# LuoGroup2023/PanTax

Measured on AMD Instinct MI355X. Metric: PAO wall-time (s) + Mreads/s: packed reads + DB (graphs and their unique-trio index) resident in HBM -> abundance tables; the metric's own GAF -> abundance quantity is value_gaf_to_tables (files -> tables, never `value`), higher is better.
Workload: dtype int64+f64

## Files before the change

include/pantax_hip.h:

```cpp
#ifndef PANTAX_HIP_H
#define PANTAX_HIP_H
#include <stddef.h>
#include <stdint.h>
#ifdef __cplusplus
extern "C" {
#endif

typedef enum {
    PANTAX_HIP_OK = 0,
    PANTAX_HIP_E_INVALID = -1,
    PANTAX_HIP_E_HIP = -2,
    PANTAX_HIP_E_NO_DEVICE = -3,
    PANTAX_HIP_E_LIMIT = -4,
    PANTAX_HIP_E_SOLVER = -5,
    PANTAX_HIP_E_IO = -6,
    PANTAX_HIP_E_STATE = -7
} pantax_hip_status;

typedef struct pantax_hip_ctx pantax_hip_ctx;
typedef struct pantax_hip_db pantax_hip_db;
typedef struct pantax_hip_reads pantax_hip_reads;

int pantax_hip_init(pantax_hip_ctx **out, const int *device_ids, int n_devices);
void pantax_hip_destroy(pantax_hip_ctx *ctx);
int pantax_hip_set_option(pantax_hip_ctx *ctx, const char *name, const char *value);
const char *pantax_hip_last_error(const pantax_hip_ctx *ctx);
const char *pantax_hip_version(void);

typedef struct {
    uint32_t n_species;
    const int64_t *range_start;
    const int64_t *range_end;
    const uint64_t *node_off;
    const int64_t *node_len;
    const uint64_t *hap_off;
    const uint64_t *path_off;
    const uint32_t *path_nodes;
} pantax_hip_graphs;

int pantax_hip_db_upload(pantax_hip_ctx *ctx, const pantax_hip_graphs *g, pantax_hip_db **out);
// ... 229 lines not shown
```

pantax_amd/_ffi.py:

```python
import ctypes as C
import os

import numpy as np

_HERE = os.path.dirname(os.path.abspath(__file__))
LIB_PATH = os.path.join(_HERE, "lib", "libpantax_hip.so")
_lib = None

SYMBOLS = [
    "pantax_hip_init", "pantax_hip_destroy", "pantax_hip_last_error", "pantax_hip_version", "pantax_hip_set_option",
    "pantax_hip_db_upload", "pantax_hip_db_upload_parts", "pantax_hip_db_free", "pantax_hip_reads_upload", "pantax_hip_reads_free",
    "pantax_hip_bin_reads", "pantax_hip_species_profile", "pantax_hip_db_reset", "pantax_hip_abundance_filter",
    "pantax_hip_trio_index", "pantax_hip_trio_get", "pantax_hip_node_coverage",
    "pantax_hip_strain_profile", "pantax_hip_strain_node_stats", "pantax_hip_strain_hap_stats", "pantax_hip_pao_solve", "pantax_hip_pao_solve_batch", "pantax_hip_profile", "pantax_hip_profile_step", "pantax_hip_profile_step_enqueue", "pantax_hip_profile_step_collect", "pantax_hip_trio_index_prefetch", "pantax_hip_sort_rows",
    "pantax_hip_sample_ranks", "pantax_hip_chacha_block", "pantax_hip_gaf_filter", "pantax_hip_db_save_images", "pantax_hip_db_load_images",
    "pantax_hip_gaf_load", "pantax_hip_gaf_load_device", "pantax_hip_reads_load_gaf", "pantax_hip_reads_set_flags", "pantax_hip_gaf_view", "pantax_hip_gaf_free",
    "pantax_hip_graph_load", "pantax_hip_graph_view", "pantax_hip_graph_free", "pantax_hip_format_f64",
    "pantax_hip_read_strains", "pantax_hip_reads_route_pack", "pantax_hip_route_buffer", "pantax_hip_route_free", "pantax_hip_reads_from_routed",
    "pantax_hip_timing_enable", "pantax_hip_timing_filter", "pantax_hip_timing_reset", "pantax_hip_timing_get", "pantax_hip_sync",
]


class PantaxHipError(RuntimeError):
    def __init__(self, code, msg):
        super().__init__("pantax_hip error %d: %s" % (code, msg))
# ... 73 lines not shown
ALLREDUCE_FN = C.CFUNCTYPE(C.c_int, C.c_void_p, C.POINTER(C.c_double), C.c_uint64)
ALLTOALLV_FN = C.CFUNCTYPE(C.c_int, C.c_void_p, C.c_void_p, C.POINTER(C.c_uint64), C.c_void_p, C.POINTER(C.c_uint64))


def load():
    global _lib
    if _lib is None:
        path = os.environ.get("PANTAX_HIP_LIB") or LIB_PATH
        if not os.path.exists(path):
            raise ImportError("%s is not built (run `python -c 'import __graft_entry__ as g; g.build()'`); "
                              "pantax_amd has no CPU fallback" % path)
        _lib = C.CDLL(path)
        _lib.pantax_hip_last_error.restype = C.c_char_p
        _lib.pantax_hip_last_error.argtypes = [C.c_void_p]
        _lib.pantax_hip_version.restype = C.c_char_p
        _lib.pantax_hip_destroy.restype = None
        _lib.pantax_hip_db_free.restype = None
        _lib.pantax_hip_reads_free.restype = None
        _lib.pantax_hip_gaf_free.restype = None
        _lib.pantax_hip_graph_free.restype = None
        _lib.pantax_hip_route_free.restype = None
        _lib.pantax_hip_read_strains.restype = C.c_int
        _lib.pantax_hip_read_strains.argtypes = [C.c_void_p, C.c_void_p, C.c_void_p, C.POINTER(ReadStrainSet), C.c_void_p, C.c_void_p, C.c_void_p]
    return _lib


def p(a):
    return None if a is None else a.ctypes.data_as(C.c_void_p)


# ... 3 lines not shown
```

pantax_amd/csrc/common.hpp:

```cpp
#pragma once
#include <hip/hip_runtime.h>
#include <cstdint>
#include <cstdio>
#include <map>
#include <functional>
#include <mutex>
#include <cstring>
#include <atomic>
#include <string>
#include <vector>
#include "../../include/pantax_hip.h"

#ifndef TRIO_LH_PACK
#define TRIO_LH_PACK 0
#endif
namespace ptx {

struct Ctx;
#if TRIO_LH_PACK
using trio_len_t = uint2;
#else
using trio_len_t = uint32_t;
#endif

// ... 101 lines not shown
    std::string cov_long;
    int covl_shape = -1;
    bool cov_count = false;
    int cov_clean_async = -1;
    bool cov_self_clean = false;
    bool walk_sum_in_bin = false;
    int ncs_prefix_min = 48;
    bool ncs_no_prefix = false;
    bool cov_arena_verify = false;
    int cov_item_groups = 0;
    int tv_u = 4, tv_rounds = 4, tf_u = 8, tf_rounds = 1, rows_u = 1, tb_slots = 256, trio_xcd = 3, cov_shape = -1, covf_shape = -1, cov_xcd = 0, group_bucket_bits = 0;
    uint32_t tv_ablate = 0, cov_ablate = 0, ssn_ablate = 0;
    bool trio_two_pass = false;
    std::string bin_route;
    std::string node_pass;
    bool no_absent_skip = false;
    bool ssn_debug = false, scan_no_huge = false, flag_rank_chained = false, ratio_kernel = false, mask_pass = false, trio_free_at_filter = false,
         trio_after_step = false;
};
int ctx_set_option(CtxConfig &cfg, const char *name, const char *value);

struct NumaInfo {
    int node = -1;
    std::vector<int> cpus;
};

struct Ctx {
    std::recursive_mutex mu;
    CtxConfig cfg;
    NumaInfo numa;
// ... 422 lines not shown
```

pantax_amd/csrc/ctx.cpp:

```cpp
#include <exception>
#include <cstdarg>
#include <algorithm>
#include <atomic>
#include <cstring>
#include <functional>
#include <chrono>
#include <condition_variable>
#include <cstdio>
#include <mutex>
#include <thread>
#include <unistd.h>
#include <fcntl.h>
#include <sched.h>
#include <pthread.h>
#include <sys/syscall.h>
#include <fstream>
#include <cctype>
#include <cstddef>
#include <cstdlib>
#include "common.hpp"

namespace ptx {

static thread_local std::string g_init_err;
static thread_local std::string g_thread_err;
static thread_local const Ctx *g_thread_err_ctx = nullptr;

int fail(Ctx *ctx, int code, const char *fmt, ...) {
    char buf[1024];
    va_list ap;
    va_start(ap, fmt);
    vsnprintf(buf, sizeof(buf), fmt, ap);
    va_end(ap);
    if (ctx) {
        { std::lock_guard<std::mutex> g(ctx->err_mu); ctx->err = buf; }
// ... 45 lines not shown
    ctx->pending.clear();
    return 0;
}

namespace {
enum OptKind { O_BOOL, O_INT, O_U32, O_U64, O_STR };
struct OptDesc { const char *name; OptKind kind; size_t off; };
#define OPT(nm, kind, field) {nm, kind, offsetof(CtxConfig, field)}
const OptDesc OPTIONS[] = {
    OPT("hip_trace", O_BOOL, trace), OPT("stage_threads", O_INT, stage_threads), OPT("stage_ch_mb", O_INT, stage_ch_mb), OPT("stream_prio", O_BOOL, stream_prio), OPT("numa_bind", O_BOOL, numa_bind), OPT("dev_cache_gb", O_INT, dev_cache_gb),
    OPT("gaf_piece_bytes", O_U64, gaf_piece_bytes), OPT("db_path_steps_max", O_U64, db_path_steps_max), OPT("db_groups", O_INT, db_groups), OPT("trio_path", O_STR, trio_path), OPT("trio_rows", O_STR, trio_rows), OPT("trio_two_pass", O_BOOL, trio_two_pass), OPT("uniq_hash", O_INT, uniq_hash),
    OPT("mask", O_STR, mask), OPT("row_sort", O_STR, row_sort), OPT("objective", O_STR, objective), OPT("read_strain_route", O_STR, read_strain_route),
    OPT("cov_general", O_BOOL, cov_general), OPT("cov_long", O_STR, cov_long), OPT("covl_shape", O_INT, covl_shape), OPT("cov_count", O_BOOL, cov_count), OPT("cov_self_clean", O_BOOL, cov_self_clean), OPT("cov_clean_async", O_INT, cov_clean_async), OPT("cov_arena_verify", O_BOOL, cov_arena_verify), OPT("ncs_no_prefix", O_BOOL, ncs_no_prefix), OPT("ncs_prefix_min", O_INT, ncs_prefix_min), OPT("walk_sum_in_bin", O_BOOL, walk_sum_in_bin), OPT("cov_item_groups", O_INT, cov_item_groups), OPT("tv_u", O_INT, tv_u), OPT("tv_rounds", O_INT, tv_rounds), OPT("tf_u", O_INT, tf_u), OPT("tf_rounds", O_INT, tf_rounds),
    OPT("rows_u", O_INT, rows_u), OPT("tb_slots", O_INT, tb_slots), OPT("trio_xcd", O_INT, trio_xcd), OPT("cov_shape", O_INT, cov_shape),
    OPT("covf_shape", O_INT, covf_shape), OPT("cov_xcd", O_INT, cov_xcd), OPT("group_bucket_bits", O_INT, group_bucket_bits), OPT("tv_ablate", O_U32, tv_ablate),
    OPT("cov_ablate", O_U32, cov_ablate), OPT("ssn_ablate", O_U32, ssn_ablate), OPT("no_absent_skip", O_BOOL, no_absent_skip), OPT("node_pass", O_STR, node_pass), OPT("bin_route", O_STR, bin_route), OPT("ssn_debug", O_BOOL, ssn_debug),
    OPT("scan_no_huge", O_BOOL, scan_no_huge), OPT("flag_rank_chained", O_BOOL, flag_rank_chained), OPT("ratio_kernel", O_BOOL, ratio_kernel),
    OPT("mask_pass", O_BOOL, mask_pass), OPT("trio_free_at_filter", O_BOOL, trio_free_at_filter), OPT("trio_after_step", O_BOOL, trio_after_step),
};
#undef OPT
}

int ctx_set_option(CtxConfig &cfg, const char *name, const char *value) {
    if (!name) return PANTAX_HIP_E_INVALID;
    static const CtxConfig defaults;
    for (const OptDesc &o : OPTIONS) {
        if (std::strcmp(o.name, name) != 0) continue;
        char *dst = reinterpret_cast<char *>(&cfg) + o.off;
        const char *def = reinterpret_cast<const char *>(&defaults) + o.off;
        char *end = nullptr;
        switch (o.kind) {
// ... 20 lines not shown

}

using namespace ptx;

extern "C" {

const char *pantax_hip_version(void) { return "pantax-hip 0.1.0 (gfx950)"; }

int pantax_hip_set_option(pantax_hip_ctx *ctx, const char *name, const char *value) {
    if (!ctx || !name) return PANTAX_HIP_E_INVALID;
    std::lock_guard<std::recursive_mutex> ptx_lock__(ctx->mu);
    const int rc = ctx_set_option(ctx->cfg, name, value);
    if (rc == 0 && std::strcmp(name, "dev_cache_gb") == 0) dev_cache_set_max(ctx->cfg.dev_cache_gb < 0 ? -1 : (long long)ctx->cfg.dev_cache_gb << 30);
    return rc == 0 ? 0 : fail(ctx, rc, "set_option: unknown option or unparsable value: %s=%s", name, value ? value : "(default)");
}

const char *pantax_hip_last_error(const pantax_hip_ctx *ctx) {
    if (!ctx) return g_init_err.c_str();
    if (g_thread_err_ctx == ctx) return g_thread_err.c_str();
    std::lock_guard<std::mutex> g(const_cast<pantax_hip_ctx *>(ctx)->err_mu);
    g_thread_err = ctx->err;
    return g_thread_err.c_str();
}

int pantax_hip_init(pantax_hip_ctx **out, const int *device_ids, int n_devices) {
    if (!out) return PANTAX_HIP_E_INVALID;
    *out = nullptr;
    if (n_devices != 1) return fail(nullptr, PANTAX_HIP_E_INVALID, "one ctx drives one GPU (one process per GPU); n_devices=%d", n_devices);
    int count = 0;
// ... 551 lines not shown
```

pantax_amd/csrc/lad.hpp:

```cpp
#pragma once
#include "common.hpp"

namespace ptx {

int hap_trio_stats_launch(Ctx *ctx, Db *db, DevBuf<uint32_t> &d_ntrio_nz , DevBuf<double> &d_mean ,
                          const uint8_t *d_active = nullptr );
int node_stats_launch(Ctx *ctx, Db *db, LadBatch *lb, int64_t min_depth, const uint8_t *d_active = nullptr);
struct RowRoute {
    uint64_t max_vs;
    uint32_t max_haps;
    bool wide;
    bool by_node;
    bool use_nodes;
    bool use_sample;
    bool ratio_by_node;
    bool masks_in_sort;
};
RowRoute row_route(const Ctx *ctx, const Db *db);
int row_pack_shift(const RowRoute &rt, uint32_t S, int pmax_bound);
bool node_pass_fused_eligible(const Ctx *ctx, const Db *db, const pantax_hip_strain_config *cfg);
int row_sample_apply(Ctx *ctx, const Db *db, LadBatch *lb, int64_t sample_nodes);
int lad_prepare(Ctx *ctx, Db *db, LadBatch *lb, bool cand_on_device, int pmax_bound);
int lad_solve_launch(Ctx *ctx, const Db *db, LadBatch *lb, int pmax_bound, const uint8_t *d_need, const uint8_t *d_fixed, double *d_x,
                     double *d_obj, int32_t *d_status, int32_t *d_iters);
struct FilterCfg;
int lad_pair_launch(Ctx *ctx, const Db *db, LadBatch *lb, int pmax_bound, const FilterCfg &fc);
int objective_launch(Ctx *ctx, const Db *db, LadBatch *lb, const uint8_t *d_need2, const double *d_x1, const double *d_x2, double *d_obj1, double *d_obj2);
struct FilterCfg { double fr, fc, sr; int shift; };
int first_filter_launch(Ctx *ctx, const Db *db, LadBatch *lb, const uint8_t *d_active, const FilterCfg &fc);

int strain_prezero(Ctx *ctx, Db *db);
int strain_enqueue(Ctx *ctx, Db *db, const pantax_hip_strain_config *cfg, const uint8_t *d_active, int slot);
int strain_finish(Ctx *ctx, Db *db, const pantax_hip_strain_config *cfg, const uint8_t *species_active, const double *species_coverage,
                  pantax_hip_hap_metrics *met, pantax_hip_solve_info *info_out, void (*after_wait)(void *), void *after_wait_arg, int slot);
int trio_index_build(Ctx *ctx, Db *db, bool with_keys);
// ... 3 lines not shown
```

pantax_amd/csrc/stage_lad.hip:

```cpp
#include <algorithm>
#include <cstdio>
#include <vector>
#include "lad.hpp"
#include "lad_device.hpp"
#include "second_filter.hpp"
#include "primitives.hpp"
#include "wave.hpp"

namespace ptx {

__device__ __forceinline__ uint32_t lower_bound_a(const double *__restrict__ a, uint32_t lo, uint32_t hi, double v) {
    while (lo < hi) { uint32_t m = (lo + hi) >> 1; if (a[m] < v) lo = m + 1; else hi = m; }
    return lo;
}
__device__ __forceinline__ uint32_t upper_bound_a(const double *__restrict__ a, uint32_t lo, uint32_t hi, double v) {
    while (lo < hi) { uint32_t m = (lo + hi) >> 1; if (a[m] <= v) lo = m + 1; else hi = m; }
    return lo;
}
__device__ __forceinline__ uint32_t wave_bound(const double *__restrict__ a, uint32_t lo, uint32_t hi, double v, bool upper) {
    const uint32_t lane = threadIdx.x & 63;
    while (hi - lo > 64) {
        const uint32_t m = hi - lo;
        const uint32_t pj = lo + (uint32_t)(((uint64_t)(lane + 1) * m) / 65);
        const double x = a[pj];
// ... 45 lines not shown
            const uint32_t jj = coop ? wave_bound(r.idx, j0, j1, v, upper)
                                     : (upper ? upper_bound_a(r.idx, j0, j1, v) : lower_bound_a(r.idx, j0, j1, v));
            if (jj > j0) lo = r.row0 + ((jj - 1) << r.shift) + 1;
            if (jj < j1) hi = r.row0 + (jj << r.shift);
        }
    }
    if (coop) return wave_bound(r.a, lo, hi, v, upper);
    return upper ? upper_bound_a(r.a, lo, hi, v) : lower_bound_a(r.a, lo, hi, v);
}
__device__ __forceinline__ uint32_t lb(bool coop, const RowIdx &r, uint32_t lo, uint32_t hi, double v) { return bound_idx(coop, r, lo, hi, v, false); }
__device__ __forceinline__ uint32_t ub_(bool coop, const RowIdx &r, uint32_t lo, uint32_t hi, double v) { return bound_idx(coop, r, lo, hi, v, true); }

constexpr int LAD_BLOCK = 256;
constexpr int LAD_KWIDE = 16;
constexpr int LAD_KLDS = 256;
enum { C_LB = 0, C_UB = 1, C_PAT = 2, C_FIXED = 3 };

#ifdef LAD_PROFILE
#define LAD_TICK(ph) do { if (tid == 0 && A.prof) { const unsigned long long now_ = wall_clock64(); A.prof[(size_t)s * 16 + (ph)] += now_ - t_prev_; \
                                                     A.prof[(size_t)s * 16 + 8 + (ph)] += 1; t_prev_ = now_; } } while (0)
#else
#define LAD_TICK(ph) do { } while (0)
#endif
struct LadArgs {
    unsigned long long *prof;
    const double *row_a;
    const uint64_t *pat_mask;
    const uint32_t *pat_start;
    const uint32_t *sp_pat_off;
    double *pat_eps, *sc_s, *sc_rho;
// ... 57 lines not shown
                off += n;                                                                                                  \
            }                                                                                                              \
            L_coff[k1 - k0] = off;                                                                                         \
        }                                                                                                                  \
        __syncthreads();                                                                                                   \
        const uint32_t total = L_coff[k1 - k0];                                                                            \
        for (uint32_t e = tid; e < total; e += LAD_BLOCK) {                                                                \
            uint32_t kk = 0, kh = k1 - k0;     \
            while (kh - kk > 1) { const uint32_t km_ = (kk + kh) >> 1; if (L_coff[km_] <= e) kk = km_; else kh = km_; }         \
            L_cache[e] = ra.a[L_crow0[kk] + (e - L_coff[kk])];                                                             \
        }                                                                                                                  \
        __syncthreads();                                                                                                   \
        cached = true;                                                                                                     \
    }
#define PAT_LOOP(k) for (uint32_t k = k0 + (COOP ? (uint32_t)(tid >> 6) : (uint32_t)tid); k < k1; k += (COOP ? LAD_BLOCK / 64 : LAD_BLOCK))
template <int PS, int NW>
struct LadLds {
    static constexpr uint32_t IDX_N = PS <= 16 ? 4096 : 2048;
    static constexpr bool CACHE_IN_G = NW == 1 && PS > 16;
    static constexpr uint32_t CACHE_N = PS <= 16 ? 2048 : CACHE_IN_G ? PS * 2 * PS : 512;
    LadShared<PS> sh;
    double W[NW == 1 ? PS * PS : 1];
    double G[NW == 1 ? PS * 2 * PS : 1];
    double L_s[LAD_KLDS], L_rho[LAD_KLDS], L_eps[LAD_KLDS];
    uint64_t L_mask[LAD_KLDS];
    uint32_t L_lo[LAD_KLDS], L_up[LAD_KLDS], L_lslo[LAD_KLDS], L_lshi[LAD_KLDS], L_lsmid[LAD_KLDS], L_start[LAD_KLDS + 1];
    double L_idx[IDX_N];
    double L_cache[CACHE_IN_G ? 1 : CACHE_N];
    uint32_t L_lsmid2[LAD_KLDS], L_coff[LAD_KLDS + 1], L_cn[LAD_KLDS], L_crow0[LAD_KLDS];
    uint32_t W_cmin[LAD_KWIDE][64], W_cmax[LAD_KWIDE][64];
    double W_acc[LAD_BLOCK / 64][2][64];
};

template <int PS, bool USEL, int NW>
__device__ __forceinline__ void lad_solve_body(const LadArgs &A, LadLds<PS, NW> &m, const int s, const int p, const uint32_t k0, const uint32_t k1) {
    static_assert(NW == 1 || !USEL, "wide species keep their pattern state in global scratch");
    constexpr uint32_t IDX_N = LadLds<PS, NW>::IDX_N, CACHE_N = LadLds<PS, NW>::CACHE_N;
    constexpr bool HUGE = NW == 0;
    const int nw = HUGE ? (int)A.wide_nw[s] : NW;
    const int ps = HUGE ? 64 * nw : PS;
    LadShared<PS> &sh = m.sh;
    double *W, *G;
    const uint64_t *patw = nullptr;
    double *q_x, *q_c, *q_d, *q_ub, *q_fac, *q_score, *q_deriv;
    long long *q_g;
    int *q_type, *q_jk, *q_dir;
    uint32_t *q_i0, *q_i1;
    if constexpr (NW == 1) { W = m.W; G = m.G; }
    else {
        const uint64_t wo = A.wide_woff[A.wide_slot[s]];
        W = A.wide_W + wo; G = A.wide_G + 2 * wo;
        patw = A.pat_or + (size_t)A.wide_off[s] * LAD_WIDE_NW;
// ... 3 lines not shown
        int *i32 = A.huge_i32 + (size_t)A.wide_coff[A.wide_slot[s]] * 5;
        q_x = f; q_c = f + ps; q_d = f + 2 * ps; q_ub = f + 3 * ps; q_fac = f + 4 * ps; q_score = f + 5 * ps; q_deriv = f + 6 * ps;
        q_g = reinterpret_cast<long long *>(f + 7 * (size_t)ps);
        q_type = i32; q_jk = i32 + ps; q_dir = i32 + 2 * ps;
        q_i0 = reinterpret_cast<uint32_t *>(i32 + 3 * (size_t)ps); q_i1 = reinterpret_cast<uint32_t *>(i32 + 4 * (size_t)ps);
    } else {
        q_x = sh.x; q_c = sh.c; q_d = sh.d; q_ub = sh.ub; q_fac = sh.fac; q_score = sh.score; q_deriv = sh.deriv; q_g = sh.g;
        q_type = sh.act_type; q_jk = sh.act_jk; q_dir = sh.dir; q_i0 = sh.act_i0; q_i1 = sh.act_i1;
    }
    auto slot_of_pattern = [&](uint32_t k) -> int {
        if constexpr (HUGE) return A.pat_act[k];
        else { int ai = -1; for (int i = 0; i < p; ++i) if (q_type[i] == C_PAT && (uint32_t)q_jk[i] == k) ai = i; return ai; }
    };
    const uint64_t c0 = A.col_off[s];
    double *L_s = m.L_s, *L_rho = m.L_rho, *L_eps = m.L_eps, *L_idx = m.L_idx, *L_cache;
    if constexpr (LadLds<PS, NW>::CACHE_IN_G) L_cache = m.G; else L_cache = m.L_cache;
    uint64_t *L_mask = m.L_mask;
    uint32_t *L_lo = m.L_lo, *L_up = m.L_up, *L_lslo = m.L_lslo, *L_lshi = m.L_lshi, *L_lsmid = m.L_lsmid, *L_start = m.L_start,
             *L_lsmid2 = m.L_lsmid2, *L_coff = m.L_coff, *L_cn = m.L_cn, *L_crow0 = m.L_crow0;
    uint32_t (*W_cmin)[64] = m.W_cmin, (*W_cmax)[64] = m.W_cmax;
    double (*W_acc)[2][64] = m.W_acc;
    const int tid = threadIdx.x;
    const bool COOP = (k1 - k0) <= (uint32_t)LAD_KWIDE;
    const bool leader = COOP ? ((tid & 63) == 0) : true;
    constexpr bool useL = USEL;
    const uint32_t kofs = useL ? k0 : 0u;
    double *P_sc_s = useL ? L_s : A.sc_s, *P_sc_rho = useL ? L_rho : A.sc_rho, *P_pat_eps = useL ? L_eps : A.pat_eps;
    uint32_t *P_sc_lo = useL ? L_lo : A.sc_lo, *P_sc_up = useL ? L_up : A.sc_up, *P_ls_lo = useL ? L_lslo : A.ls_lo,
             *P_ls_hi = useL ? L_lshi : A.ls_hi, *P_ls_mid = useL ? L_lsmid : A.ls_mid;
    const uint64_t *P_pat_mask = useL ? L_mask : A.pat_mask;
    const uint32_t *P_pat_start = useL ? L_start : A.pat_start;
// ... 641 lines not shown
        if (v > q_ub[j]) v = q_ub[j];
        A.x_out[c0 + j] = v;
    }
    if (tid == 0) {
        A.status[s] = (it >= max_it) ? 1 : sh.status;
        A.iters[s] = it;
    }
}

template <int NW>
__device__ __forceinline__ bool lad_instance_takes(const LadArgs &A, int s, int p) {
    if (NW == 1) return p <= LAD_MAXP;
    if (p <= LAD_MAXP) return false;
    return (NW == 0) == (A.wide_nw[s] > (uint32_t)LAD_WIDE_NW);
}
template <int PS, int NW>
__global__ void __launch_bounds__(LAD_BLOCK) lad_solve_kernel(LadArgs A) {
    __shared__ LadLds<PS, NW> m;
    const int s = NW == 1 ? (int)blockIdx.x : (int)A.wide_list[blockIdx.x];
    const int p = A.sp_p[s];
    if (!lad_instance_takes<NW>(A, s, p)) return;
    if (A.need && !A.need[s]) return;
    if (p <= 0) { if (threadIdx.x == 0) { A.status[s] = 0; A.iters[s] = 0; } return; }
    const uint32_t k0 = A.sp_pat_off[s], k1 = A.sp_pat_off[s + 1];
    if constexpr (NW == 1) {
        if (k1 - k0 <= (uint32_t)LAD_KLDS) lad_solve_body<PS, true, 1>(A, m, s, p, k0, k1);
        else lad_solve_body<PS, false, 1>(A, m, s, p, k0, k1);
    } else lad_solve_body<PS, false, NW>(A, m, s, p, k0, k1);
}

template <int PS, int NW>
__global__ void __launch_bounds__(LAD_BLOCK) lad_pair_kernel(LadArgs A1, LadArgs A2, SecondFilterArgs F) {
    __shared__ LadLds<PS, NW> m;
    const int s = NW == 1 ? (int)blockIdx.x : (int)A1.wide_list[blockIdx.x];
    const int p = A1.sp_p[s];
    if (!lad_instance_takes<NW>(A1, s, p)) return;
    const uint32_t k0 = A1.sp_pat_off[s], k1 = A1.sp_pat_off[s + 1];
    const bool lds_state = NW == 1 && k1 - k0 <= (uint32_t)LAD_KLDS;
    if (p > 0) {
        if constexpr (NW == 1) {
            if (lds_state) lad_solve_body<PS, true, 1>(A1, m, s, p, k0, k1);
            else lad_solve_body<PS, false, 1>(A1, m, s, p, k0, k1);
        } else lad_solve_body<PS, false, NW>(A1, m, s, p, k0, k1);
    } else if (threadIdx.x == 0) { A1.status[s] = 0; A1.iters[s] = 0; }
    __syncthreads();
    if (threadIdx.x == 0) second_filter_species(F, (uint32_t)s);
    __syncthreads();
    if (p <= 0 || !F.need2[s]) return;
    if constexpr (NW == 1) {
        if (lds_state) lad_solve_body<PS, true, 1>(A2, m, s, p, k0, k1);
        else lad_solve_body<PS, false, 1>(A2, m, s, p, k0, k1);
    } else lad_solve_body<PS, false, NW>(A2, m, s, p, k0, k1);
}

static SecondFilterArgs second_filter_args(const Db *db, LadBatch *lb, const FilterCfg &fc, const double *d_x1, const int32_t *d_status1,
                                           uint8_t *d_fixed2, uint8_t *d_need2) {
    SecondFilterArgs F;
    F.hap_off = db->d_hap_off.p; F.hap_nt = lb->d_hap_nt.p; F.sp_trio = lb->d_sp_trio.p; F.hap_bit = lb->d_hap_bit.p; F.sp_p = lb->d_p.p; F.nnz = db->d_hap_nnz.p;
    F.meanf = db->d_hap_mean.p; F.ratio = lb->d_ratio.p; F.x1 = d_x1; F.status1 = d_status1; F.fc = fc.fc; F.sr = fc.sr;
    F.fixed2 = d_fixed2; F.need2 = d_need2;
    return F;
}
static LadArgs lad_args(const Db *db, LadBatch *lb, const uint8_t *d_need, const uint8_t *d_fixed, double *d_x, int32_t *d_status, int32_t *d_iters) {
    LadArgs A;
    A.prof = nullptr;
    A.row_a = lb->row_a; A.pat_mask = lb->d_pat_mask.p; A.pat_start = lb->d_pat_start.p; A.sp_pat_off = lb->d_sp_pat_off.p;
    A.pat_eps = lb->d_pat_eps.p; A.sc_s = lb->d_sc_s.p; A.sc_rho = lb->d_sc_rho.p;
// ... 25 lines not shown
    for (uint32_t s = 0; s < S && s < 4; ++s) {
        unsigned long long tot = 0;
        for (int ph = 0; ph < 8; ++ph) tot += h[(size_t)s * 16 + ph];
        if (!tot) continue;
        std::fprintf(stderr, "[lad profile] species %u: %d pivots, %.1f us in the pivot loop (%.1f us per pivot)\n", s, it[s], tot * 0.01, it[s] ? tot * 0.01 / it[s] : 0.0);
        for (int ph = 0; ph < 8; ++ph)
            std::fprintf(stderr, "    %-22s %9.1f us  %5.1f %%  (%llu visits, %.2f us each)\n", LAD_PHASE_NAMES[ph], h[(size_t)s * 16 + ph] * 0.01,
                         100.0 * h[(size_t)s * 16 + ph] / tot, h[(size_t)s * 16 + 8 + ph], h[(size_t)s * 16 + 8 + ph] ? h[(size_t)s * 16 + ph] * 0.01 / h[(size_t)s * 16 + 8 + ph] : 0.0);
    }
    return 0;
}
#endif

int lad_pair_launch(Ctx *ctx, const Db *db, LadBatch *lb, int pmax_bound, const FilterCfg &fc) {
    const uint32_t S = db->S;
    LadArgs A1 = lad_args(db, lb, nullptr, nullptr, lb->d_x.p, lb->d_status.p, lb->d_iters.p);
    LadArgs A2 = lad_args(db, lb, nullptr, lb->d_fixed2.p, lb->d_x2.p, lb->d_status2.p, lb->d_iters2.p);
    SecondFilterArgs F = second_filter_args(db, lb, fc, lb->d_x.p, lb->d_status.p, lb->d_fixed2.p, lb->d_need2.p);
#ifdef LAD_PROFILE
    DevBuf<unsigned long long> prof;
    PTX_TRY(lad_prof_begin(ctx, S, prof, A1));
#endif
    {
        KTimer t(ctx, "lad_pair_kernel");
        if (pmax_bound <= 16) hipLaunchKernelGGL((lad_pair_kernel<16, 1>), dim3(S), dim3(LAD_BLOCK), 0, ctx->stream, A1, A2, F);
        else hipLaunchKernelGGL((lad_pair_kernel<LAD_MAXP, 1>), dim3(S), dim3(LAD_BLOCK), 0, ctx->stream, A1, A2, F);
        if (lb->n_wide > lb->n_huge) hipLaunchKernelGGL((lad_pair_kernel<LAD_WIDEP, LAD_WIDE_NW>), dim3(lb->n_wide), dim3(LAD_BLOCK), 0, ctx->stream, A1, A2, F);
        if (lb->n_huge) hipLaunchKernelGGL((lad_pair_kernel<1, 0>), dim3(lb->n_wide), dim3(LAD_BLOCK), 0, ctx->stream, A1, A2, F);
    }
    PTX_HIP(ctx, hipGetLastError());
#ifdef LAD_PROFILE
    PTX_TRY(lad_prof_end(ctx, S, prof, lb->d_iters.p));
#endif
    return objective_launch(ctx, db, lb, lb->d_need2.p, lb->d_x.p, lb->d_x2.p, lb->d_obj.p, lb->d_obj2.p);
}

int lad_solve_launch(Ctx *ctx, const Db *db, LadBatch *lb, int pmax_bound, const uint8_t *d_need, const uint8_t *d_fixed, double *d_x,
                     double *d_obj, int32_t *d_status, int32_t *d_iters) {
    const uint32_t S = db->S;
    LadArgs A = lad_args(db, lb, d_need, d_fixed, d_x, d_status, d_iters);
#ifdef LAD_PROFILE
    DevBuf<unsigned long long> prof;
    PTX_TRY(lad_prof_begin(ctx, S, prof, A));
#endif
    {
        KTimer t(ctx, "lad_solve_kernel");
        if (pmax_bound <= 16) hipLaunchKernelGGL((lad_solve_kernel<16, 1>), dim3(S), dim3(LAD_BLOCK), 0, ctx->stream, A);
        else hipLaunchKernelGGL((lad_solve_kernel<LAD_MAXP, 1>), dim3(S), dim3(LAD_BLOCK), 0, ctx->stream, A);
        if (lb->n_wide > lb->n_huge) hipLaunchKernelGGL((lad_solve_kernel<LAD_WIDEP, LAD_WIDE_NW>), dim3(lb->n_wide), dim3(LAD_BLOCK), 0, ctx->stream, A);
        if (lb->n_huge) hipLaunchKernelGGL((lad_solve_kernel<1, 0>), dim3(lb->n_wide), dim3(LAD_BLOCK), 0, ctx->stream, A);
    }
    PTX_HIP(ctx, hipGetLastError());
#ifdef LAD_PROFILE
    PTX_TRY(lad_prof_end(ctx, S, prof, d_iters));
#endif
    return objective_launch(ctx, db, lb, nullptr, d_x, nullptr, d_obj, nullptr);
}

}
```

pantax_amd/csrc/stage_lp_rows.hip:

```cpp
#include <algorithm>
#include <cstdio>
#include <vector>
#include "lad.hpp"
#include "lad_device.hpp"
#include "primitives.hpp"
#include "wave.hpp"
#include "scan_chained.hpp"

namespace ptx {

__device__ __forceinline__ uint32_t find_hap_l(const uint64_t *__restrict__ path_off, uint32_t H, uint64_t q) {
    uint32_t lo = 0, hi = H;
    while (lo < hi) { uint32_t mid = (lo + hi) >> 1; if (path_off[mid] <= q) lo = mid + 1; else hi = mid; }
    return lo - 1;
}

__global__ void __launch_bounds__(256) mask_kernel(const uint2 *__restrict__ tiles, const uint64_t *__restrict__ path_off,
                                                   const uint32_t *__restrict__ path_nodes, const uint32_t *__restrict__ hap_species,
                                                   const uint32_t *__restrict__ node_base, const int32_t *__restrict__ hap_bit,
                                                   unsigned long long *__restrict__ mask, const int32_t *__restrict__ sp_p,
                                                   const uint32_t *__restrict__ wide_off ,
                                                   const uint32_t *__restrict__ wide_nw, unsigned long long *__restrict__ maskw,
                                                   const uint64_t *__restrict__ by_node_hap_off ) {
    const uint2 tile = tiles[blockIdx.x];
// ... 440 lines not shown
        if (ev[0] == 'n') r.use_nodes = r.max_vs <= SSN_MAX_SEG && S <= 65535 && V > 0;
    }
    r.use_sample = V <= SS_MAX_N;
    r.by_node = use_node_haps(ctx, db);
    r.ratio_by_node = r.by_node && V && !ctx->cfg.ratio_kernel;
    r.wide = max_hs > (uint64_t)LAD_MAXP;
    const bool mask_pass_env = ctx->cfg.mask_pass || ctx->cfg.objective == "nodes";
    r.masks_in_sort = r.use_nodes && r.ratio_by_node && !db->nh_walk_too && !r.wide && !mask_pass_env;
    return r;
}
int row_pack_shift(const RowRoute &rt, uint32_t S, int pmax_bound) {
    const int sp_bits = S > 1 ? bits_for(S - 1) : 0;
    return (!rt.use_sample && sp_bits + pmax_bound <= 64 && !(rt.use_nodes && pmax_bound >= 64)) ? pmax_bound : -1;
}

bool node_pass_fused_eligible(const Ctx *ctx, const Db *db, const pantax_hip_strain_config *cfg) {
    if (ctx->cfg.node_pass == "split" || !db->cov_count_pending || db->V == 0) return false;
    if (cfg->sample_nodes != 0 || ctx->cfg.cov_self_clean || db->cov_self_clean) return false;
    if (db->L / db->V >= (uint64_t)ctx->cfg.ncs_prefix_min && !ctx->cfg.ncs_no_prefix) return false;
    return row_route(ctx, db).masks_in_sort;
}

static int upload_candidates(Ctx *ctx, const Db *db, LadBatch *lb) {
    const uint32_t S = db->S;
    const uint64_t H = db->H;
    std::vector<int32_t> hap_bit(H ? H : 1, -1);
    for (uint32_t s = 0; s < S; ++s)
        for (int k = 0; k < lb->h_p[s]; ++k) hap_bit[db->h_hap_off[s] + lb->h_cand[db->h_hap_off[s] + k]] = k;
    PTX_TRY(upload(ctx, lb->d_hap_bit, hap_bit.data(), hap_bit.size()));
    PTX_TRY(upload(ctx, lb->d_p, lb->h_p.data(), S));
// ... 195 lines not shown
```

pantax_amd/engine.py:

```python
import ctypes as C

import numpy as np

from . import _ffi
from ._ffi import PantaxHipError, as_c, p


class Engine:
    def __init__(self, device=0):
        self.lib = _ffi.load()
        self.ctx = C.c_void_p()
        dev = (C.c_int * 1)(device)
        rc = self.lib.pantax_hip_init(C.byref(self.ctx), dev, 1)
        if rc != 0:
            raise PantaxHipError(rc, self.lib.pantax_hip_last_error(None).decode())
        self.db = None
        self.reads = None
        self._keep = []
        self._step_buf = None
        self._collect_buf = None
        self._inflight = 0

    def _check(self, rc):
        if rc != 0:
# ... 21 lines not shown
                self.lib.pantax_hip_db_free(self.ctx, self.db)
                self.db = None
            self._inflight = 0

    def __enter__(self):
        return self

    def __exit__(self, *a):
        self.close()

    def sync(self):
        self._check(self.lib.pantax_hip_sync(self.ctx))

    def set_option(self, name, value=None):
        self._check(self.lib.pantax_hip_set_option(self.ctx, name.encode(), None if value is None else str(value).encode()))

    def upload_db(self, species):
        if self.db:
            self.lib.pantax_hip_db_free(self.ctx, self.db)
            self.db = None
            self._inflight = 0
        S = len(species)
        self.S = S
        self.range_start = as_c([g.range_start for g in species], np.int64)
        self.range_end = as_c([g.range_end for g in species], np.int64)
        self.node_off = np.zeros(S + 1, dtype=np.uint64)
        self.node_off[1:] = np.cumsum([len(g.node_len) for g in species])
        self.hap_off = np.zeros(S + 1, dtype=np.uint64)
        self.hap_off[1:] = np.cumsum([len(g.path_off) - 1 for g in species])
        self.V = int(self.node_off[-1])
# ... 476 lines not shown
```

Baseline: 6284.

## Add compact LDS shape for 16-column LAD solver when species exceed CUs

Adds a second shared-memory layout for the 16-column LAD solver kernels with smaller index, cache and per-pattern LDS arrays plus a waves-per-EU hint of 4. By default it is chosen automatically when there are more species workgroups than compute units, so several workgroups can share a CU instead of one large-LDS block each. The trade-off is that species with more than 32 patterns fall back to the global-memory state path, and index and cache capacity shrink, which may cost extra global traffic. An option and a query function expose the choice.

```diff
diff --git a/include/pantax_hip.h b/include/pantax_hip.h
--- a/include/pantax_hip.h
+++ b/include/pantax_hip.h
@@ -24,6 +24,7 @@
 int pantax_hip_init(pantax_hip_ctx **out, const int *device_ids, int n_devices);
 void pantax_hip_destroy(pantax_hip_ctx *ctx);
 int pantax_hip_set_option(pantax_hip_ctx *ctx, const char *name, const char *value);
+const char *pantax_hip_lad_shape_name(const pantax_hip_ctx *ctx, uint32_t n_species, int max_columns);
 const char *pantax_hip_last_error(const pantax_hip_ctx *ctx);
 const char *pantax_hip_version(void);
 
diff --git a/pantax_amd/_ffi.py b/pantax_amd/_ffi.py
--- a/pantax_amd/_ffi.py
+++ b/pantax_amd/_ffi.py
@@ -8,7 +8,7 @@
 _lib = None
 
 SYMBOLS = [
-    "pantax_hip_init", "pantax_hip_destroy", "pantax_hip_last_error", "pantax_hip_version", "pantax_hip_set_option",
+    "pantax_hip_init", "pantax_hip_destroy", "pantax_hip_last_error", "pantax_hip_version", "pantax_hip_set_option", "pantax_hip_lad_shape_name",
     "pantax_hip_db_upload", "pantax_hip_db_upload_parts", "pantax_hip_db_free", "pantax_hip_reads_upload", "pantax_hip_reads_free",
     "pantax_hip_bin_reads", "pantax_hip_species_profile", "pantax_hip_db_reset", "pantax_hip_abundance_filter",
     "pantax_hip_trio_index", "pantax_hip_trio_get", "pantax_hip_node_coverage",
@@ -112,6 +112,8 @@
         _lib.pantax_hip_last_error.restype = C.c_char_p
         _lib.pantax_hip_last_error.argtypes = [C.c_void_p]
         _lib.pantax_hip_version.restype = C.c_char_p
+        _lib.pantax_hip_lad_shape_name.restype = C.c_char_p
+        _lib.pantax_hip_lad_shape_name.argtypes = [C.c_void_p, C.c_uint32, C.c_int]
         _lib.pantax_hip_destroy.restype = None
         _lib.pantax_hip_db_free.restype = None
         _lib.pantax_hip_reads_free.restype = None
diff --git a/pantax_amd/csrc/common.hpp b/pantax_amd/csrc/common.hpp
--- a/pantax_amd/csrc/common.hpp
+++ b/pantax_amd/csrc/common.hpp
@@ -139,6 +139,7 @@
     bool trio_two_pass = false;
     std::string bin_route;
     std::string node_pass;
+    std::string lad_shape;
     bool no_absent_skip = false;
     bool ssn_debug = false, scan_no_huge = false, flag_rank_chained = false, ratio_kernel = false, mask_pass = false, trio_free_at_filter = false,
          trio_after_step = false;
diff --git a/pantax_amd/csrc/ctx.cpp b/pantax_amd/csrc/ctx.cpp
--- a/pantax_amd/csrc/ctx.cpp
+++ b/pantax_amd/csrc/ctx.cpp
@@ -19,6 +19,7 @@
 #include <cstddef>
 #include <cstdlib>
 #include "common.hpp"
+#include "lad.hpp"
 
 namespace ptx {
 
@@ -94,7 +95,7 @@
     OPT("cov_general", O_BOOL, cov_general), OPT("cov_long", O_STR, cov_long), OPT("covl_shape", O_INT, covl_shape), OPT("cov_count", O_BOOL, cov_count), OPT("cov_self_clean", O_BOOL, cov_self_clean), OPT("cov_clean_async", O_INT, cov_clean_async), OPT("cov_arena_verify", O_BOOL, cov_arena_verify), OPT("ncs_no_prefix", O_BOOL, ncs_no_prefix), OPT("ncs_prefix_min", O_INT, ncs_prefix_min), OPT("walk_sum_in_bin", O_BOOL, walk_sum_in_bin), OPT("cov_item_groups", O_INT, cov_item_groups), OPT("tv_u", O_INT, tv_u), OPT("tv_rounds", O_INT, tv_rounds), OPT("tf_u", O_INT, tf_u), OPT("tf_rounds", O_INT, tf_rounds),
     OPT("rows_u", O_INT, rows_u), OPT("tb_slots", O_INT, tb_slots), OPT("trio_xcd", O_INT, trio_xcd), OPT("cov_shape", O_INT, cov_shape),
     OPT("covf_shape", O_INT, covf_shape), OPT("cov_xcd", O_INT, cov_xcd), OPT("group_bucket_bits", O_INT, group_bucket_bits), OPT("tv_ablate", O_U32, tv_ablate),
-    OPT("cov_ablate", O_U32, cov_ablate), OPT("ssn_ablate", O_U32, ssn_ablate), OPT("no_absent_skip", O_BOOL, no_absent_skip), OPT("node_pass", O_STR, node_pass), OPT("bin_route", O_STR, bin_route), OPT("ssn_debug", O_BOOL, ssn_debug),
+    OPT("cov_ablate", O_U32, cov_ablate), OPT("ssn_ablate", O_U32, ssn_ablate), OPT("no_absent_skip", O_BOOL, no_absent_skip), OPT("node_pass", O_STR, node_pass), OPT("bin_route", O_STR, bin_route), OPT("lad_shape", O_STR, lad_shape), OPT("ssn_debug", O_BOOL, ssn_debug),
     OPT("scan_no_huge", O_BOOL, scan_no_huge), OPT("flag_rank_chained", O_BOOL, flag_rank_chained), OPT("ratio_kernel", O_BOOL, ratio_kernel),
     OPT("mask_pass", O_BOOL, mask_pass), OPT("trio_free_at_filter", O_BOOL, trio_free_at_filter), OPT("trio_after_step", O_BOOL, trio_after_step),
 };
@@ -145,6 +146,11 @@
     const int rc = ctx_set_option(ctx->cfg, name, value);
     if (rc == 0 && std::strcmp(name, "dev_cache_gb") == 0) dev_cache_set_max(ctx->cfg.dev_cache_gb < 0 ? -1 : (long long)ctx->cfg.dev_cache_gb << 30);
     return rc == 0 ? 0 : fail(ctx, rc, "set_option: unknown option or unparsable value: %s=%s", name, value ? value : "(default)");
+}
+
+const char *pantax_hip_lad_shape_name(const pantax_hip_ctx *ctx, uint32_t n_species, int max_columns) {
+    if (!ctx) return nullptr;
+    return lad_shape_name(lad_shape(ctx->cfg.lad_shape, n_species, ctx->n_cu, max_columns));
 }
 
 const char *pantax_hip_last_error(const pantax_hip_ctx *ctx) {
diff --git a/pantax_amd/csrc/lad.hpp b/pantax_amd/csrc/lad.hpp
--- a/pantax_amd/csrc/lad.hpp
+++ b/pantax_amd/csrc/lad.hpp
@@ -19,6 +19,9 @@
 RowRoute row_route(const Ctx *ctx, const Db *db);
 int row_pack_shift(const RowRoute &rt, uint32_t S, int pmax_bound);
 bool node_pass_fused_eligible(const Ctx *ctx, const Db *db, const pantax_hip_strain_config *cfg);
+enum class LadShape { roomy, compact };
+LadShape lad_shape(const std::string &option, uint32_t n_workgroups, int n_cu, int pmax_bound);
+const char *lad_shape_name(LadShape s);
 int row_sample_apply(Ctx *ctx, const Db *db, LadBatch *lb, int64_t sample_nodes);
 int lad_prepare(Ctx *ctx, Db *db, LadBatch *lb, bool cand_on_device, int pmax_bound);
 int lad_solve_launch(Ctx *ctx, const Db *db, LadBatch *lb, int pmax_bound, const uint8_t *d_need, const uint8_t *d_fixed, double *d_x,
diff --git a/pantax_amd/csrc/stage_lad.hip b/pantax_amd/csrc/stage_lad.hip
--- a/pantax_amd/csrc/stage_lad.hip
+++ b/pantax_amd/csrc/stage_lad.hip
@@ -83,6 +83,9 @@
 constexpr int LAD_BLOCK = 256;
 constexpr int LAD_KWIDE = 16;
 constexpr int LAD_KLDS = 256;
+
+struct LadRoomy { static constexpr uint32_t IDX_N = 4096, CACHE_N = 2048; static constexpr int KLDS = LAD_KLDS, WAVES = 1; };
+struct LadCompact { static constexpr uint32_t IDX_N = 1024, CACHE_N = 1024; static constexpr int KLDS = 32, WAVES = 4; };
 enum { C_LB = 0, C_UB = 1, C_PAT = 2, C_FIXED = 3 };
 
 #ifdef LAD_PROFILE
@@ -170,28 +173,30 @@
         cached = true;                                                                                                     \
     }
 #define PAT_LOOP(k) for (uint32_t k = k0 + (COOP ? (uint32_t)(tid >> 6) : (uint32_t)tid); k < k1; k += (COOP ? LAD_BLOCK / 64 : LAD_BLOCK))
-template <int PS, int NW>
+template <int PS, int NW, class SH = LadRoomy>
 struct LadLds {
-    static constexpr uint32_t IDX_N = PS <= 16 ? 4096 : 2048;
+    static_assert(PS <= 16 || SH::KLDS == LAD_KLDS, "only the 16-column instance has more than one shape");
+    static constexpr int KLDS = SH::KLDS;
+    static constexpr uint32_t IDX_N = PS <= 16 ? SH::IDX_N : 2048;
     static constexpr bool CACHE_IN_G = NW == 1 && PS > 16;
-    static constexpr uint32_t CACHE_N = PS <= 16 ? 2048 : CACHE_IN_G ? PS * 2 * PS : 512;
+    static constexpr uint32_t CACHE_N = PS <= 16 ? SH::CACHE_N : CACHE_IN_G ? PS * 2 * PS : 512;
     LadShared<PS> sh;
     double W[NW == 1 ? PS * PS : 1];
     double G[NW == 1 ? PS * 2 * PS : 1];
-    double L_s[LAD_KLDS], L_rho[LAD_KLDS], L_eps[LAD_KLDS];
-    uint64_t L_mask[LAD_KLDS];
-    uint32_t L_lo[LAD_KLDS], L_up[LAD_KLDS], L_lslo[LAD_KLDS], L_lshi[LAD_KLDS], L_lsmid[LAD_KLDS], L_start[LAD_KLDS + 1];
+    double L_s[KLDS], L_rho[KLDS], L_eps[KLDS];
+    uint64_t L_mask[KLDS];
+    uint32_t L_lo[KLDS], L_up[KLDS], L_lslo[KLDS], L_lshi[KLDS], L_lsmid[KLDS], L_start[KLDS + 1];
     double L_idx[IDX_N];
     double L_cache[CACHE_IN_G ? 1 : CACHE_N];
-    uint32_t L_lsmid2[LAD_KLDS], L_coff[LAD_KLDS + 1], L_cn[LAD_KLDS], L_crow0[LAD_KLDS];
+    uint32_t L_lsmid2[KLDS], L_coff[KLDS + 1], L_cn[KLDS], L_crow0[KLDS];
     uint32_t W_cmin[LAD_KWIDE][64], W_cmax[LAD_KWIDE][64];
     double W_acc[LAD_BLOCK / 64][2][64];
 };
 
-template <int PS, bool USEL, int NW>
-__device__ __forceinline__ void lad_solve_body(const LadArgs &A, LadLds<PS, NW> &m, const int s, const int p, const uint32_t k0, const uint32_t k1) {
+template <int PS, bool USEL, int NW, class SH>
+__device__ __forceinline__ void lad_solve_body(const LadArgs &A, LadLds<PS, NW, SH> &m, const int s, const int p, const uint32_t k0, const uint32_t k1) {
     static_assert(NW == 1 || !USEL, "wide species keep their pattern state in global scratch");
-    constexpr uint32_t IDX_N = LadLds<PS, NW>::IDX_N, CACHE_N = LadLds<PS, NW>::CACHE_N;
+    constexpr uint32_t IDX_N = LadLds<PS, NW, SH>::IDX_N, CACHE_N = LadLds<PS, NW, SH>::CACHE_N;
     constexpr bool HUGE = NW == 0;
     const int nw = HUGE ? (int)A.wide_nw[s] : NW;
     const int ps = HUGE ? 64 * nw : PS;
@@ -225,7 +230,7 @@
     };
     const uint64_t c0 = A.col_off[s];
     double *L_s = m.L_s, *L_rho = m.L_rho, *L_eps = m.L_eps, *L_idx = m.L_idx, *L_cache;
-    if constexpr (LadLds<PS, NW>::CACHE_IN_G) L_cache = m.G; else L_cache = m.L_cache;
+    if constexpr (LadLds<PS, NW, SH>::CACHE_IN_G) L_cache = m.G; else L_cache = m.L_cache;
     uint64_t *L_mask = m.L_mask;
     uint32_t *L_lo = m.L_lo, *L_up = m.L_up, *L_lslo = m.L_lslo, *L_lshi = m.L_lshi, *L_lsmid = m.L_lsmid, *L_start = m.L_start,
              *L_lsmid2 = m.L_lsmid2, *L_coff = m.L_coff, *L_cn = m.L_cn, *L_crow0 = m.L_crow0;
@@ -897,9 +902,9 @@
     if (p <= LAD_MAXP) return false;
     return (NW == 0) == (A.wide_nw[s] > (uint32_t)LAD_WIDE_NW);
 }
-template <int PS, int NW>
-__global__ void __launch_bounds__(LAD_BLOCK) lad_solve_kernel(LadArgs A) {
-    __shared__ LadLds<PS, NW> m;
+template <int PS, int NW, class SH = LadRoomy>
+__global__ void __launch_bounds__(LAD_BLOCK) __attribute__((amdgpu_waves_per_eu(SH::WAVES))) lad_solve_kernel(LadArgs A) {
+    __shared__ LadLds<PS, NW, SH> m;
     const int s = NW == 1 ? (int)blockIdx.x : (int)A.wide_list[blockIdx.x];
     const int p = A.sp_p[s];
     if (!lad_instance_takes<NW>(A, s, p)) return;
@@ -907,33 +912,41 @@
     if (p <= 0) { if (threadIdx.x == 0) { A.status[s] = 0; A.iters[s] = 0; } return; }
     const uint32_t k0 = A.sp_pat_off[s], k1 = A.sp_pat_off[s + 1];
     if constexpr (NW == 1) {
-        if (k1 - k0 <= (uint32_t)LAD_KLDS) lad_solve_body<PS, true, 1>(A, m, s, p, k0, k1);
-        else lad_solve_body<PS, false, 1>(A, m, s, p, k0, k1);
-    } else lad_solve_body<PS, false, NW>(A, m, s, p, k0, k1);
-}
-
-template <int PS, int NW>
-__global__ void __launch_bounds__(LAD_BLOCK) lad_pair_kernel(LadArgs A1, LadArgs A2, SecondFilterArgs F) {
-    __shared__ LadLds<PS, NW> m;
+        if (k1 - k0 <= (uint32_t)SH::KLDS) lad_solve_body<PS, true, 1, SH>(A, m, s, p, k0, k1);
+        else lad_solve_body<PS, false, 1, SH>(A, m, s, p, k0, k1);
+    } else lad_solve_body<PS, false, NW, SH>(A, m, s, p, k0, k1);
+}
+
+template <int PS, int NW, class SH = LadRoomy>
+__global__ void __launch_bounds__(LAD_BLOCK) __attribute__((amdgpu_waves_per_eu(SH::WAVES))) lad_pair_kernel(LadArgs A1, LadArgs A2, SecondFilterArgs F) {
+    __shared__ LadLds<PS, NW, SH> m;
     const int s = NW == 1 ? (int)blockIdx.x : (int)A1.wide_list[blockIdx.x];
     const int p = A1.sp_p[s];
     if (!lad_instance_takes<NW>(A1, s, p)) return;
     const uint32_t k0 = A1.sp_pat_off[s], k1 = A1.sp_pat_off[s + 1];
-    const bool lds_state = NW == 1 && k1 - k0 <= (uint32_t)LAD_KLDS;
+    const bool lds_state = NW == 1 && k1 - k0 <= (uint32_t)SH::KLDS;
     if (p > 0) {
         if constexpr (NW == 1) {
-            if (lds_state) lad_solve_body<PS, true, 1>(A1, m, s, p, k0, k1);
-            else lad_solve_body<PS, false, 1>(A1, m, s, p, k0, k1);
-        } else lad_solve_body<PS, false, NW>(A1, m, s, p, k0, k1);
+            if (lds_state) lad_solve_body<PS, true, 1, SH>(A1, m, s, p, k0, k1);
+            else lad_solve_body<PS, false, 1, SH>(A1, m, s, p, k0, k1);
+        } else lad_solve_body<PS, false, NW, SH>(A1, m, s, p, k0, k1);
     } else if (threadIdx.x == 0) { A1.status[s] = 0; A1.iters[s] = 0; }
     __syncthreads();
     if (threadIdx.x == 0) second_filter_species(F, (uint32_t)s);
     __syncthreads();
     if (p <= 0 || !F.need2[s]) return;
     if constexpr (NW == 1) {
-        if (lds_state) lad_solve_body<PS, true, 1>(A2, m, s, p, k0, k1);
-        else lad_solve_body<PS, false, 1>(A2, m, s, p, k0, k1);
-    } else lad_solve_body<PS, false, NW>(A2, m, s, p, k0, k1);
+        if (lds_state) lad_solve_body<PS, true, 1, SH>(A2, m, s, p, k0, k1);
+        else lad_solve_body<PS, false, 1, SH>(A2, m, s, p, k0, k1);
+    } else lad_solve_body<PS, false, NW, SH>(A2, m, s, p, k0, k1);
+}
+
+static int lad_shape_checked(Ctx *ctx, uint32_t S, int pmax_bound, LadShape *out) {
+    const std::string &opt = ctx->cfg.lad_shape;
+    if (!opt.empty() && opt != "auto" && opt != "roomy" && opt != "compact")
+        return fail(ctx, PANTAX_HIP_E_INVALID, "lad solver: option lad_shape is \"auto\", \"roomy\" or \"compact\", not \"%s\"", opt.c_str());
+    *out = lad_shape(opt, S, ctx->n_cu, pmax_bound);
+    return 0;
 }
 
 static SecondFilterArgs second_filter_args(const Db *db, LadBatch *lb, const FilterCfg &fc, const double *d_x1, const int32_t *d_status1,
@@ -989,6 +1002,8 @@
 
 int lad_pair_launch(Ctx *ctx, const Db *db, LadBatch *lb, int pmax_bound, const FilterCfg &fc) {
     const uint32_t S = db->S;
+    LadShape shape;
+    PTX_TRY(lad_shape_checked(ctx, S, pmax_bound, &shape));
     LadArgs A1 = lad_args(db, lb, nullptr, nullptr, lb->d_x.p, lb->d_status.p, lb->d_iters.p);
     LadArgs A2 = lad_args(db, lb, nullptr, lb->d_fixed2.p, lb->d_x2.p, lb->d_status2.p, lb->d_iters2.p);
     SecondFilterArgs F = second_filter_args(db, lb, fc, lb->d_x.p, lb->d_status.p, lb->d_fixed2.p, lb->d_need2.p);
@@ -998,7 +1013,8 @@
 #endif
     {
         KTimer t(ctx, "lad_pair_kernel");
-        if (pmax_bound <= 16) hipLaunchKernelGGL((lad_pair_kernel<16, 1>), dim3(S), dim3(LAD_BLOCK), 0, ctx->stream, A1, A2, F);
+        if (shape == LadShape::compact) hipLaunchKernelGGL((lad_pair_kernel<16, 1, LadCompact>), dim3(S), dim3(LAD_BLOCK), 0, ctx->stream, A1, A2, F);
+        else if (pmax_bound <= 16) hipLaunchKernelGGL((lad_pair_kernel<16, 1>), dim3(S), dim3(LAD_BLOCK), 0, ctx->stream, A1, A2, F);
         else hipLaunchKernelGGL((lad_pair_kernel<LAD_MAXP, 1>), dim3(S), dim3(LAD_BLOCK), 0, ctx->stream, A1, A2, F);
         if (lb->n_wide > lb->n_huge) hipLaunchKernelGGL((lad_pair_kernel<LAD_WIDEP, LAD_WIDE_NW>), dim3(lb->n_wide), dim3(LAD_BLOCK), 0, ctx->stream, A1, A2, F);
         if (lb->n_huge) hipLaunchKernelGGL((lad_pair_kernel<1, 0>), dim3(lb->n_wide), dim3(LAD_BLOCK), 0, ctx->stream, A1, A2, F);
@@ -1013,6 +1029,8 @@
 int lad_solve_launch(Ctx *ctx, const Db *db, LadBatch *lb, int pmax_bound, const uint8_t *d_need, const uint8_t *d_fixed, double *d_x,
                      double *d_obj, int32_t *d_status, int32_t *d_iters) {
     const uint32_t S = db->S;
+    LadShape shape;
+    PTX_TRY(lad_shape_checked(ctx, S, pmax_bound, &shape));
     LadArgs A = lad_args(db, lb, d_need, d_fixed, d_x, d_status, d_iters);
 #ifdef LAD_PROFILE
     DevBuf<unsigned long long> prof;
@@ -1020,7 +1038,8 @@
 #endif
     {
         KTimer t(ctx, "lad_solve_kernel");
-        if (pmax_bound <= 16) hipLaunchKernelGGL((lad_solve_kernel<16, 1>), dim3(S), dim3(LAD_BLOCK), 0, ctx->stream, A);
+        if (shape == LadShape::compact) hipLaunchKernelGGL((lad_solve_kernel<16, 1, LadCompact>), dim3(S), dim3(LAD_BLOCK), 0, ctx->stream, A);
+        else if (pmax_bound <= 16) hipLaunchKernelGGL((lad_solve_kernel<16, 1>), dim3(S), dim3(LAD_BLOCK), 0, ctx->stream, A);
         else hipLaunchKernelGGL((lad_solve_kernel<LAD_MAXP, 1>), dim3(S), dim3(LAD_BLOCK), 0, ctx->stream, A);
         if (lb->n_wide > lb->n_huge) hipLaunchKernelGGL((lad_solve_kernel<LAD_WIDEP, LAD_WIDE_NW>), dim3(lb->n_wide), dim3(LAD_BLOCK), 0, ctx->stream, A);
         if (lb->n_huge) hipLaunchKernelGGL((lad_solve_kernel<1, 0>), dim3(lb->n_wide), dim3(LAD_BLOCK), 0, ctx->stream, A);
diff --git a/pantax_amd/csrc/stage_lp_rows.hip b/pantax_amd/csrc/stage_lp_rows.hip
--- a/pantax_amd/csrc/stage_lp_rows.hip
+++ b/pantax_amd/csrc/stage_lp_rows.hip
@@ -478,6 +478,13 @@
     return (!rt.use_sample && sp_bits + pmax_bound <= 64 && !(rt.use_nodes && pmax_bound >= 64)) ? pmax_bound : -1;
 }
 
+LadShape lad_shape(const std::string &option, uint32_t n_workgroups, int n_cu, int pmax_bound) {
+    if (pmax_bound > 16 || option == "roomy") return LadShape::roomy;
+    if (option == "compact") return LadShape::compact;
+    return n_workgroups > (uint32_t)std::max(n_cu, 0) ? LadShape::compact : LadShape::roomy;
+}
+const char *lad_shape_name(LadShape s) { return s == LadShape::compact ? "compact" : "roomy"; }
+
 bool node_pass_fused_eligible(const Ctx *ctx, const Db *db, const pantax_hip_strain_config *cfg) {
     if (ctx->cfg.node_pass == "split" || !db->cov_count_pending || db->V == 0) return false;
     if (cfg->sample_nodes != 0 || ctx->cfg.cov_self_clean || db->cov_self_clean) return false;
diff --git a/pantax_amd/engine.py b/pantax_amd/engine.py
--- a/pantax_amd/engine.py
+++ b/pantax_amd/engine.py
@@ -59,6 +59,9 @@
 
     def set_option(self, name, value=None):
         self._check(self.lib.pantax_hip_set_option(self.ctx, name.encode(), None if value is None else str(value).encode()))
+
+    def lad_shape_name(self, n_species, max_columns):
+        return self.lib.pantax_hip_lad_shape_name(self.ctx, int(n_species), int(max_columns)).decode()
 
     def upload_db(self, species):
         if self.db:
```

After: 6447, median of 6. +2.6%, better.
